# ruuda/robigo-luculenta

Hardware: AMD Instinct MI355X
Metric: Mrays/sec on built-in scene at 1920x1080 (higher is better)
Workload: dtype f32

## Files before the change

### robigo_luculenta_amd/csrc/rl_core.h

```cpp
#pragma once
#include "rl_math.h"
#include "rl_rng.h"
#include "rl_scene.h"

#if defined(__HIP_DEVICE_COMPILE__) && !defined(__gfx950__)
#error "rl_core.h's device fast paths (64-bit ballots, two scratch slots per lane, ds_bpermute batches) are written for wave64 gfx950"
#endif

struct RlF3 {
    float x, y, z;
};
RL_HD RlF3 rl_f3(float x, float y, float z) {
    RlF3 r;
    r.x = x;
    r.y = y;
    r.z = z;
    return r;
}
RL_HD RlF3 rl_add(RlF3 a, RlF3 b) { return rl_f3(a.x + b.x, a.y + b.y, a.z + b.z); }
RL_HD RlF3 rl_sub(RlF3 a, RlF3 b) { return rl_f3(a.x - b.x, a.y - b.y, a.z - b.z); }
RL_HD RlF3 rl_neg(RlF3 a) { return rl_f3(-a.x, -a.y, -a.z); }
RL_HD RlF3 rl_mul(RlF3 a, float f) { return rl_f3(a.x * f, a.y * f, a.z * f); }
RL_HD float rl_dot(RlF3 a, RlF3 b) { return a.x * b.x + a.y * b.y + a.z * b.z; }
RL_HD RlF3 rl_cross(RlF3 a, RlF3 b) {
// ... 61 lines not shown
RL_HD RlF3 rl_xyz(RlF4 v) { return rl_f3(v.x, v.y, v.z); }

struct RlQuat {
    float x, y, z, w;
};
RL_HD RlQuat rl_qmul(RlQuat a, RlQuat b) {
    RlQuat r;
    r.x = a.w * b.x + a.x * b.w + a.y * b.z - a.z * b.y;
    r.y = a.w * b.y - a.x * b.z + a.y * b.w + a.z * b.x;
    r.z = a.w * b.z + a.x * b.y - a.y * b.x + a.z * b.w;
    r.w = a.w * b.w - a.x * b.x - a.y * b.y - a.z * b.z;
    return r;
}
RL_HD RlF3 rl_qrotate(RlF3 v, RlQuat q) {
    RlQuat p;
    p.x = v.x; p.y = v.y; p.z = v.z; p.w = 0.0f;
    RlQuat c;
    c.x = -q.x; c.y = -q.y; c.z = -q.z; c.w = q.w;
    const RlQuat r = rl_qmul(rl_qmul(q, p), c);
    return rl_f3(r.x, r.y, r.z);
}


struct RlPath {
    RlF3 origin, direction;
    float wavelength;
    float intensity;
    float continue_chance;
    float sx, sy;
    float ior;
    uint32_t bounce;
};

enum { RL_HIT_NONE = 0xffffffffu };

struct RlHit {
    float t;
    uint32_t obj;
    uint32_t sub;
};

RL_HD float rl_sf10_ior(float wavelength) {
    const double w2 = (double)(wavelength * wavelength * 1.0e-6f);
#if defined(__HIP_DEVICE_COMPILE__)
    {
        const double t1 = w2 - 0.0131887070, t2 = w2 - 0.0623068142, t3 = w2 - 155.23629000;
        const double t23 = t2 * t3, t13 = t1 * t3, t12 = t1 * t2;
        const double num = __builtin_fma(1.737596950 * w2, t23, __builtin_fma(0.313747346 * w2, t13, (1.898781010 * w2) * t12));
        const double den = t1 * t23;
        double y = __builtin_amdgcn_rcp(den);
        y = __builtin_fma(y, __builtin_fma(-den, y, 1.0), y);
        y = __builtin_fma(y, __builtin_fma(-den, y, 1.0), y);
        const double sum = 1.0 + num * y;
        double r = __builtin_amdgcn_rsq(sum);
        r = __builtin_fma(0.5 * r, __builtin_fma(-(sum * r), r, 1.0), r);
        r = __builtin_fma(0.5 * r, __builtin_fma(-(sum * r), r, 1.0), r);
        const double n = sum * r;
        const float lo = (float)(n * (1.0 - 9.094947017729282e-13)), hi = (float)(n * (1.0 + 9.094947017729282e-13));
        if (RL_LIKELY(__builtin_amdgcn_ballot_w64(!(lo == hi)) == 0)) return lo;
    }
#endif
    return (float)sqrt(1.0 + 1.737596950 * w2 / (w2 - 0.0131887070) + 0.313747346 * w2 / (w2 - 0.0623068142) +
                       1.898781010 * w2 / (w2 - 155.23629000));
}


RL_HD void rl_begin_path(const RlSceneView& sv, float aspect_ratio, uint64_t seed, uint32_t stream, uint64_t path,
                         RlPath* p) {
    const RlRngBlock b0 = rl_rng_block(seed, stream, path, 0);
    const float wavelength = rl_get_wavelength(b0.w[0]);
    const float x = rl_get_bi_unit(b0.w[1]);
    const float y = rl_get_bi_unit(b0.w[2]) / aspect_ratio;
    const float t = rl_get_unit(b0.w[3]);

    const float* crec = (const float*)sv.camera_rec;
    RlCameraDesc cd;
    cd.phi0 = crec[0]; cd.phi1 = crec[1]; cd.alpha0 = crec[2]; cd.alpha1 = crec[3]; cd.dist0 = crec[4]; cd.dist1 = crec[5];
    cd.fov_over_pi = crec[6]; cd.focal_factor = crec[7]; cd.depth_of_field = crec[8]; cd.chromatic_abberation = crec[9];
    const float screen_distance = crec[10];
    const float phi = RL_PI_F * (cd.phi0 + cd.phi1 * t);
    const float alpha = RL_PI_F * (cd.alpha0 + cd.alpha1 * t);
    const float distance = cd.dist0 + cd.dist1 * t;
    float sin_a, cos_a, sin_p, cos_p;
    rl_sincosf(alpha, &sin_a, &cos_a);
    rl_sincosf(phi, &sin_p, &cos_p);
    const RlF3 position = rl_f3(cos_a * sin_p * distance, cos_a * cos_p * distance, sin_a * distance);
    float s1, c1, s2, c2;
    rl_sincosf((phi + RL_PI_F) * 0.5f, &s1, &c1);
    rl_sincosf((-alpha) * 0.5f, &s2, &c2);
    RlQuat q1, q2;
    q1.x = s1 * 0.0f; q1.y = s1 * 0.0f; q1.z = s1 * -1.0f; q1.w = c1;
    q2.x = s2 * 1.0f; q2.y = s2 * 0.0f; q2.z = s2 * 0.0f;  q2.w = c2;
    const RlQuat orientation = rl_qmul(q1, q2);
    const float focal_distance = distance * cd.focal_factor;

    const RlRngBlock b1 = rl_rng_block(seed, stream, path, 1);
    const float dof_angle = rl_get_longitude(b1.w[0]);
    const float dof_radius = rl_get_unit(b1.w[1]) / cd.depth_of_field;
    const float d = rl_div200f(wavelength - 580.0f);
    const float zoom = 1.0f + d * cd.chromatic_abberation;

    const float xs = x * zoom;
    const float ys = y * zoom;
    const RlF3 direction = rl_normalise(rl_f3(xs, screen_distance, -ys));
    const RlF3 focus_point = rl_mul(direction, focal_distance / direction.y);
    float sin_d, cos_d;
    rl_sincosf(dof_angle, &sin_d, &cos_d);
    const RlF3 lens_point = rl_f3(cos_d * dof_radius, 0.0f, sin_d * dof_radius);

    p->origin = rl_add(position, rl_qrotate(lens_point, orientation));
    p->direction = rl_normalise(rl_qrotate(rl_sub(focus_point, lens_point), orientation));
    p->wavelength = wavelength;
    p->intensity = 1.0f;
    p->continue_chance = 1.0f;
    p->sx = x;
    p->sy = y;
    p->ior = rl_sf10_ior(wavelength);
    p->bounce = 0;
}


template <bool AXIS_Z = false>
RL_HD float rl_plane_t(RlF3 n, RlF3 off, RlF3 o, RlF3 dir, float* dn_out) {
    const RlF3 lo = rl_sub(o, off);
    const float dn = AXIS_Z ? n.z * dir.z : rl_dot(n, dir);
    *dn_out = dn;
    const float t = -(AXIS_Z ? n.z * lo.z : rl_dot(n, lo)) / dn;
    return (dn != 0.0f && t > 0.0f) ? t : -1.0f;
}
template <bool AXIS_Z = false>
RL_HD bool rl_plane_hit(RlF3 n, RlF3 off, RlF3 o, RlF3 dir, float* t_out) {
    const RlF3 lo = rl_sub(o, off);
    const float dn = AXIS_Z ? n.z * dir.z : rl_dot(n, dir);
    const float t = -(AXIS_Z ? n.z * lo.z : rl_dot(n, lo)) / dn;
    *t_out = t;
    return (dn != 0.0f) & (t > 0.0f);
}
RL_HD bool rl_inside(RlF3 n, RlF3 off, RlF3 p) { return rl_dot(rl_sub(p, off), n) < 0.0f; }

RL_HD float rl_paraboloid_roots(float a, float b, float c) {
    if (a == 0.0f) {
        const float t1 = -c / b;
        if (t1 < 0.0f) return -1.0f;
        return t1;
    }
    const float disc = b * b - 4.0f * a * c;
    if (disc < 0.0f) return -1.0f;
    const float sq = sqrtf(disc);
    const float p = 0.5f * (-b + sq) / a;
    const float q = 0.5f * (-b - sq) / a;
    if (p > 0.0f && (p < q || q < 0.0f)) return p;
    if (q > 0.0f) return q;
    return -1.0f;
}
template <bool AXIS_Z = false>
RL_HD float rl_paraboloid_t(RlF3 offset, RlF3 normal, RlF3 focal_point, RlF3 o, RlF3 dir, bool* hit_out = nullptr) {
    const RlF3 origin = rl_sub(o, offset);
    const RlF3 focal_offset = rl_sub(origin, focal_point);
    const float n_dot_d = AXIS_Z ? normal.z * dir.z : rl_dot(normal, dir);
    const float n_dot_o = AXIS_Z ? normal.z * origin.z : rl_dot(normal, origin);
    const float d_dot_f = rl_dot(dir, focal_offset);
    const float a = n_dot_d * n_dot_d - 1.0f;
    const float b = 2.0f * n_dot_d * n_dot_o - 2.0f * d_dot_f;
    const float c = n_dot_o * n_dot_o - rl_dot(focal_offset, focal_offset);
#if defined(__HIP_DEVICE_COMPILE__)
    const float disc = b * b - 4.0f * a * c;
    const float sq = rl_sqrtf(disc, true);
    const float np = -b + sq, nq = -b - sq;
    const float pick = np < 0.0f ? np : nq;
    float largest;
    asm("v_max_f32 %0, |%1|, %2" : "=v"(largest) : "v"(b), "v"(sq));
    const bool plain = (a < 0.0f) & ((disc < 0.0f) | (largest >= 8.0779356694631609e-28f));
    if (RL_LIKELY(__builtin_amdgcn_ballot_w64(!plain) == 0)) {
        const float t = 0.5f * pick / a;
        if (hit_out) {
            *hit_out = !(disc < 0.0f) & (pick < 0.0f);
            return t;
        }
        return ((disc < 0.0f) | !(pick < 0.0f)) ? -1.0f : t;
    }
#endif
    const float t_literal = rl_paraboloid_roots(a, b, c);
    if (hit_out) *hit_out = !(t_literal < 0.0f);
    return t_literal;
}

struct RlCand {
    float t;
    uint32_t k;
};
// ... 629 lines not shown
```

### robigo_luculenta_amd/csrc/rl_kernels.hip.h

```cpp
#pragma once
#include <hip/hip_runtime.h>

#include <cstddef>
#include <type_traits>

#include "rl_cie1931.h"
#include "rl_core.h"

#define RL_BLOCK 256
#ifndef RL_TRACE_BLOCK
#define RL_TRACE_BLOCK 1024
#endif
#ifndef RL_TRACE_WPS
#define RL_TRACE_WPS 4
#endif
#ifndef RL_TRACE_VGPRS
#define RL_TRACE_VGPRS (RL_TRACE_WPS == 4 ? 128 : 96)
#endif
#ifndef RL_TRACE_VGPRS_OPEN
#define RL_TRACE_VGPRS_OPEN (RL_TRACE_WPS == 4 ? 120 : 96)
#endif
#define RL_EMIT_MAX_AGE 8u
#define RL_CHUNK 256ull

// ... 1022 lines not shown
        if (pend_me) __hip_atomic_fetch_add(wg_fin + my_job, 1u, __ATOMIC_RELAXED, __HIP_MEMORY_SCOPE_WORKGROUP);
        if (lane < emit_pend)
            __hip_atomic_fetch_add(wg_fin + (((RlLdsU32*)ws->ring_b)[lane] >> 24), 1u, __ATOMIC_RELAXED,
                                   __HIP_MEMORY_SCOPE_WORKGROUP);
        pend_me = false;
        pend_any = false;
        emit_pend = 0;
    };
    auto flush = [&](uint32_t gap) {
        const uint32_t now = (uint32_t)wall_clock64();
        uint32_t mine = gap == 0u ? 1u : 0u;
        if (lane == 0 && gap != 0u) {
            uint32_t at = *wg_flushed_at;
            if (now - at >= gap)
                mine = __hip_atomic_compare_exchange_strong(wg_flushed_at, &at, now | 1u, __ATOMIC_RELAXED, __ATOMIC_RELAXED,
                                                            __HIP_MEMORY_SCOPE_WORKGROUP) ? 1u : 0u;
        }
        if (__builtin_amdgcn_readfirstlane(mine) == 0u) return;
        for (uint32_t base_job = 0; base_job < known_local; base_job += 64u) {
            const uint32_t jb = base_job + lane;
            uint32_t f = 0, sg = 0;
            if (jb < known_local) {
                f = __hip_atomic_exchange(wg_fin + jb, 0u, __ATOMIC_RELAXED, __HIP_MEMORY_SCOPE_WORKGROUP);
                sg = __hip_atomic_exchange(wg_seg + jb, 0u, __ATOMIC_RELAXED, __HIP_MEMORY_SCOPE_WORKGROUP);
            }
            if (__builtin_amdgcn_ballot_w64((f | sg) != 0u) == 0) continue;
            if (sg != 0) __hip_atomic_fetch_add(&od->seg[jb], sg, __ATOMIC_RELAXED, __HIP_MEMORY_SCOPE_AGENT);
            __builtin_amdgcn_fence(__ATOMIC_RELEASE, "workgroup");
            if (f != 0) {
                const uint32_t before = __hip_atomic_fetch_add(&od->fin[jb], f, __ATOMIC_RELAXED, __HIP_MEMORY_SCOPE_AGENT);
                if (before + f == (uint32_t)od->jobs[jb].end) {
                    __hip_atomic_fetch_add(&od->completed, 1u, __ATOMIC_RELAXED, __HIP_MEMORY_SCOPE_AGENT);
                    const uint32_t total = __hip_atomic_load(&od->seg[jb], __ATOMIC_RELAXED, __HIP_MEMORY_SCOPE_AGENT);
                    __hip_atomic_store(&ctl->segs[jb], total, __ATOMIC_RELAXED, __HIP_MEMORY_SCOPE_SYSTEM);
                    __hip_atomic_store(&ctl->done[jb], 1u, __ATOMIC_RELEASE, __HIP_MEMORY_SCOPE_SYSTEM);
                }
            }
        }
    };
    uint32_t e_head = 0, e_tail = 0;
    uint32_t emit_age = 0;
#ifdef RL_STATS
    unsigned long long st[RL_ST_COUNT];
    for (int k = 0; k < RL_ST_COUNT; ++k) st[k] = 0;
#endif
    RL_T0(t_total);

    auto process_emitted = [&](uint32_t count) {
        RL_STAT(RL_ST_EMIT_BATCHES, 1);
        RL_STAT(RL_ST_EMIT_LANES, count);
        if (OPEN && emit_pend != 0) settle();
        rl_wave_sync();
        if (!FUSED) {
            uint32_t idx = 0, tagged = 0;
            float value = 0.0f;
            RlMappedPhoton* dst_base = photons;
            if (lane < count) {
                const uint32_t slot = (e_head + lane) & 63u;
                idx = rl_f2u(emit_get(0, slot));
                tagged = rl_f2u(emit_get(4, slot));
                if (OPEN) ((RlLdsU32*)ws->ring_b)[lane] = tagged;
                uint64_t first = job.first_path;
                if (OPEN) {
                    const RlJobEntry e = jobs[tagged >> 24];
                    first = e.first_path, dst_base = (RlMappedPhoton*)e.target;
                }
                const RlRngBlock b0 = rl_rng_block(job.seed, job.stream, first + idx, 0);
                RlMappedPhoton ph;
                ph.wavelength = rl_get_wavelength(b0.w[0]);
                ph.x = rl_get_bi_unit(b0.w[1]);
                ph.y = rl_get_bi_unit(b0.w[2]) / job.aspect_ratio;
                value = rl_emission(sv, emit_get(3, slot), ph.wavelength, OPEN ? (tagged & 0xffffffu) : tagged);
                ph.probability = value;
                if (OPEN) {
                    uint32_t* dst = (uint32_t*)&dst_base[idx];
                    __hip_atomic_store(dst + 0, rl_f2u(ph.x), __ATOMIC_RELAXED, __HIP_MEMORY_SCOPE_AGENT);
                    __hip_atomic_store(dst + 1, rl_f2u(ph.y), __ATOMIC_RELAXED, __HIP_MEMORY_SCOPE_AGENT);
                    __hip_atomic_store(dst + 2, rl_f2u(ph.probability), __ATOMIC_RELAXED, __HIP_MEMORY_SCOPE_AGENT);
                    __hip_atomic_store(dst + 3, rl_f2u(ph.wavelength), __ATOMIC_RELAXED, __HIP_MEMORY_SCOPE_AGENT);
                } else {
                    dst_base[idx] = ph;
                }
            }
        } else if (lane < count) {
            const uint32_t slot = (e_head + lane) & 63u;
            const float sx = emit_get(0, slot), sy = emit_get(1, slot), wavelength = emit_get(2, slot);
            const uint32_t tagged = rl_f2u(emit_get(4, slot));
            if (OPEN) ((RlLdsU32*)ws->ring_b)[lane] = tagged;
            float* target = plot;
            if (OPEN) target = (float*)jobs[tagged >> 24].target;
            const float value = rl_emission(sv, emit_get(3, slot), wavelength, OPEN ? (tagged & 0xffffffu) : tagged);
            if (value != 0.0f) {
                const RlF3 cie = rl_mul(rl_tristimulus(sv.cie, wavelength), value);
                uint32_t width = job.width, height = job.height;
                asm volatile("" : "+s"(width), "+s"(height));
                const RlSplat sp = rl_splat_weights(width, height, job.wm1, job.hm1, job.aspect_ratio, sx, sy);
#pragma unroll
                for (int k = 0; k < 4; ++k) {
                    float* px = target + 3ull * sp.idx[k];
                    unsafeAtomicAdd(px + 0, cie.x * sp.w[k]);
                    unsafeAtomicAdd(px + 1, cie.y * sp.w[k]);
                    unsafeAtomicAdd(px + 2, cie.z * sp.w[k]);
                }
            }
        }
        if (OPEN) emit_pend = count;
        rl_wave_sync();
    };

    for (;;) {
        if (OPEN) {
            settle();
            flush(3000u);
        }
        RL_T0(t_refill);
        auto refill = [&]() -> bool {
            if (drained) return false;
                uint32_t open_n = 0;
                if (OPEN) {
                    bool got = false;
                    for (;;) {
                        if (chunk_next < chunk_end) {
                            open_n = (uint32_t)jobs[stash_job].end;
                            got = true;
                            break;
                        }
                        if (stash_job < known_local) {
                            open_n = (uint32_t)jobs[stash_job].end;
                            const uint32_t take = known_local - stash_job >= 2u ? 256u : 64u;
                            uint32_t b = 0;
                            if (lane == 0) b = __hip_atomic_fetch_add(&od->next[stash_job], take, __ATOMIC_RELAXED, __HIP_MEMORY_SCOPE_AGENT);
                            b = __builtin_amdgcn_readfirstlane(b);
                            if (b < open_n) {
                                chunk_end = b + take < open_n ? b + take : ((open_n + 63u) & ~63u);
                                chunk_next = b;
                                got = true;
                                break;
                            }
                            stash_job += 1u;
                            continue;
                        }
                        const uint32_t now = (uint32_t)wall_clock64();
                        const uint32_t seen = __builtin_amdgcn_readfirstlane(wg_poll[0]), seen_at = __builtin_amdgcn_readfirstlane(wg_poll[1]);
                        if (seen > known_local) {
                            __builtin_amdgcn_fence(__ATOMIC_ACQUIRE, "agent");
                            known_local = seen;
                            continue;
                        }
                        if (now - seen_at < 1000u) break;
                        if (lane == 0) wg_poll[1] = now;
                        uint32_t v = 0;
                        if (lane == 0) v = __hip_atomic_load(&od->known, __ATOMIC_RELAXED, __HIP_MEMORY_SCOPE_AGENT);
                        v = __builtin_amdgcn_readfirstlane(v);
                        if (v > known_local) {
                            if (lane == 0) wg_poll[0] = v;
                            __builtin_amdgcn_fence(__ATOMIC_ACQUIRE, "agent");
                            known_local = v;
                            continue;
                        }
                        if (lane == 0) v = __hip_atomic_load(&od->closed, __ATOMIC_RELAXED, __HIP_MEMORY_SCOPE_AGENT);
                        if (__builtin_amdgcn_readfirstlane(v) != 0u) {
                            drained = true;
                            break;
                        }
                        if (lane == 0) {
                            uint32_t expected = 0;
                            v = __hip_atomic_compare_exchange_strong(&od->closing, &expected, 1u, __ATOMIC_ACQUIRE, __ATOMIC_RELAXED,
                                                                     __HIP_MEMORY_SCOPE_AGENT) ? 1u : 0u;
                        }
                        if (__builtin_amdgcn_readfirstlane(v) == 0u) break;
                        uint32_t pub = 0;
                        if (lane == 0) pub = __hip_atomic_load(&ctl->published, __ATOMIC_ACQUIRE, __HIP_MEMORY_SCOPE_SYSTEM);
                        pub = __builtin_amdgcn_readfirstlane(pub);
                        if (pub > RL_OPEN_CAP) pub = RL_OPEN_CAP;
                        if (pub > known_local) {
                            for (uint32_t k = known_local + lane; k < pub; k += 64u) {
                                unsigned long long* dst = (unsigned long long*)&od->jobs[k];
                                const unsigned long long* src = (const unsigned long long*)&ctl->jobs[k];
                                for (int w = 0; w < 4; ++w)
                                    __hip_atomic_store(dst + w, __hip_atomic_load(src + w, __ATOMIC_RELAXED, __HIP_MEMORY_SCOPE_SYSTEM),
                                                       __ATOMIC_RELAXED, __HIP_MEMORY_SCOPE_AGENT);
                            }
                            __builtin_amdgcn_fence(__ATOMIC_RELEASE, "agent");
                            if (lane == 0) {
                                od->idle_since = 0;
                                od->stuck_since = 0;
                                wg_poll[0] = pub;
                                __hip_atomic_store(&od->known, pub, __ATOMIC_RELEASE, __HIP_MEMORY_SCOPE_AGENT);
                                __hip_atomic_store(&od->closing, 0u, __ATOMIC_RELEASE, __HIP_MEMORY_SCOPE_AGENT);
                            }
                            known_local = pub;
                            continue;
                        }
                        uint32_t stay = 0;
                        if (lane == 0 && known_local < RL_OPEN_CAP) {
                            const bool finishing = __hip_atomic_load(&od->completed, __ATOMIC_RELAXED, __HIP_MEMORY_SCOPE_AGENT) < known_local;
                            const unsigned long long now = wall_clock64(), since = finishing ? od->stuck_since : od->idle_since;
                            uint32_t grace = job.grace_ticks;
                            asm volatile("" : "+s"(grace));
                            const unsigned long long limit = finishing ? 500000000ull : (unsigned long long)grace;
                            if (since == 0) (finishing ? od->stuck_since : od->idle_since) = now, stay = 1;
                            else if (now - since < limit) stay = 1;
                            if (!finishing) od->stuck_since = 0;
                            if (stay) __hip_atomic_store(&od->closing, 0u, __ATOMIC_RELEASE, __HIP_MEMORY_SCOPE_AGENT);
                        }
                        if (__builtin_amdgcn_readfirstlane(stay) != 0u) break;
                        uint32_t again = 0;
                        if (lane == 0) {
                            __hip_atomic_store(&ctl->closed_at, known_local, __ATOMIC_SEQ_CST, __HIP_MEMORY_SCOPE_SYSTEM);
                            __builtin_amdgcn_fence(__ATOMIC_SEQ_CST, "");
                            again = __hip_atomic_load(&ctl->published, __ATOMIC_SEQ_CST, __HIP_MEMORY_SCOPE_SYSTEM);
                        }
                        again = __builtin_amdgcn_readfirstlane(again);
                        if (again == known_local || known_local >= RL_OPEN_CAP) {
                            if (lane == 0) {
                                __hip_atomic_store(&ctl->final_at, known_local, __ATOMIC_SEQ_CST, __HIP_MEMORY_SCOPE_SYSTEM);
                                __hip_atomic_store(&od->closed, 1u, __ATOMIC_RELEASE, __HIP_MEMORY_SCOPE_AGENT);
                            }
                            drained = true;
                            break;
                        }
                        if (lane == 0) {
                            __hip_atomic_store(&ctl->closed_at, RL_OPEN_NONE, __ATOMIC_SEQ_CST, __HIP_MEMORY_SCOPE_SYSTEM);
                            __hip_atomic_store(&od->closing, 0u, __ATOMIC_RELEASE, __HIP_MEMORY_SCOPE_AGENT);
                        }
                    }
                    if (!got) return false;
                }
                if (!OPEN && chunk_next == chunk_end) {
                    const unsigned long long chunk =
                        job.n_paths >= (unsigned long long)gridDim.x * (RL_TRACE_BLOCK * 16ull) ? RL_CHUNK : 64ull;
                    unsigned long long b = 0;
                    if (lane == 0) b = atomicAdd(&queue[0], chunk);
                    const uint32_t lo = __builtin_amdgcn_readfirstlane((uint32_t)b);
                    const uint32_t hi = __builtin_amdgcn_readfirstlane((uint32_t)(b >> 32));
                    chunk_next = ((uint64_t)hi << 32) | lo;
                    chunk_end = chunk_next + chunk;
                }
                RL_STAT(RL_ST_REFILLS, 1);
                if (OPEN) stash_first = jobs[stash_job].first_path;
                const uint64_t limit = OPEN ? (uint64_t)open_n : job.n_paths;
                stash_path0 = stash_first + chunk_next;
                stash_valid = chunk_next >= limit ? 0u : (limit - chunk_next >= 64ull ? 64u : (uint32_t)(limit - chunk_next));
                chunk_next += 64;
                const bool valid = lane < stash_valid;
                const uint64_t path_index = stash_path0 + lane;
                RlPath fresh = p;
                RL_T0(t_cam);
                if (valid) rl_begin_path(sv, job.aspect_ratio, job.seed, job.stream, path_index, &fresh);
                RL_T1(RL_ST_T_CAMERA, t_cam);
                rl_wave_sync();
                stash[0 * 64 + lane] = fresh.origin.x;
                stash[1 * 64 + lane] = fresh.origin.y;
                stash[2 * 64 + lane] = fresh.origin.z;
                stash[3 * 64 + lane] = fresh.direction.x;
                stash[4 * 64 + lane] = fresh.direction.y;
                stash[5 * 64 + lane] = fresh.direction.z;
                stash[6 * 64 + lane] = fresh.wavelength;
                stash[7 * 64 + lane] = fresh.sx;
                stash[8 * 64 + lane] = fresh.sy;
                stash[9 * 64 + lane] = fresh.ior;
                rl_wave_sync();
                stash_head = 0;
                stash_count = 64;
                if (!OPEN && chunk_next >= job.n_paths) drained = true;
            return true;
        };
        auto hand_out = [&](const uint64_t need) -> bool {
            const uint32_t avail = stash_count - stash_head;
            const uint32_t rank = rl_mbcnt(need);
            const uint32_t slot = stash_head + rank;
            const bool take = !active & (rank < avail) & (slot < stash_valid);
            {
                const uint32_t sl = slot & 63u;
                const float s0 = stash[0 * 64 + sl], s1 = stash[1 * 64 + sl], s2 = stash[2 * 64 + sl], s3 = stash[3 * 64 + sl], s4 = stash[4 * 64 + sl];
                const float s5 = stash[5 * 64 + sl], s6 = stash[6 * 64 + sl], s7 = stash[7 * 64 + sl], s8 = stash[8 * 64 + sl], s9 = stash[9 * 64 + sl];
                my_path = take ? stash_path0 + slot : my_path;
                if (OPEN) my_job = take ? stash_job : my_job;
                p.origin = rl_f3(take ? s0 : p.origin.x, take ? s1 : p.origin.y, take ? s2 : p.origin.z);
                p.direction = rl_f3(take ? s3 : p.direction.x, take ? s4 : p.direction.y, take ? s5 : p.direction.z);
                p.wavelength = take ? s6 : p.wavelength;
                p.sx = take ? s7 : p.sx;
                p.sy = take ? s8 : p.sy;
                p.ior = take ? s9 : p.ior;
                p.intensity = take ? 1.0f : p.intensity;
                p.continue_chance = take ? 1.0f : p.continue_chance;
                p.bounce = take ? 0u : p.bounce;
                active = active | take;
            }
            const uint32_t wanted = (uint32_t)__popcll(need);
            stash_head += wanted < avail ? wanted : avail;
            return wanted <= avail;
        };
        {
            const uint64_t need = __builtin_amdgcn_ballot_w64(!active);
            if (need != 0) {
                bool served = false;
                if (RL_LIKELY(stash_count != stash_head)) served = hand_out(need);
                if (RL_UNLIKELY(!served)) {
                    if (refill()) hand_out(__builtin_amdgcn_ballot_w64(!active));
                }
            }
        }
        RL_T1(RL_ST_T_REFILL, t_refill);
        if (__builtin_amdgcn_ballot_w64(active) == 0) {
            if (!OPEN || drained) break;
            settle();
            if (e_tail != e_head) {
                process_emitted(e_tail - e_head);
                e_head = e_tail;
                settle();
            }
            flush(500u);
            for (int k = 0; k < 4; ++k) __builtin_amdgcn_s_sleep(127);
            continue;
        }
        constexpr bool FULL = !OPEN || (STAGE == RL_STAGE_ALL && (FUSED || !CYL));
        const RlHit hit = rl_scan_wave<CYL, FULL, STAGE != RL_STAGE_NONE && (!(FUSED && OPEN) || FULL), STAGE != RL_STAGE_NONE && (!(OPEN && (FUSED || STAGE == RL_STAGE_TABLES)) || FULL), STAGE == RL_STAGE_ALL, STAGE != RL_STAGE_NONE, STAGE != RL_STAGE_ALL>(sv, base + (lay.off_cull - tab0), CYL ? base + (lay.off_prism_cyl - tab0) : nullptr, lay.group_gc, lay.small_ordered, lay.cull_cmax2, lay.n_cluster_groups, lay.n_prism_groups,
                                       lay.n_cluster_supers, lay.super_g, ring_t, p.origin, p.direction, active ? 0u : 0x80000000u, ws, lane RL_TACC_ARG);
#ifdef RL_STATS
        {
            const uint32_t mk = (active && hit.obj != RL_HIT_NONE) ? rl_object_material(rl_f2u(sv.objects[hit.obj].w)) : 99u;
            const uint64_t m_act = __builtin_amdgcn_ballot_w64(active);
            const uint64_t m_void = __builtin_amdgcn_ballot_w64(active && hit.obj == RL_HIT_NONE);
            const uint64_t m_emit = __builtin_amdgcn_ballot_w64(mk == RL_MATERIAL_BLACK_BODY);
            const uint64_t m_grey = __builtin_amdgcn_ballot_w64(mk == RL_MATERIAL_DIFFUSE_GREY);
            const uint64_t m_col = __builtin_amdgcn_ballot_w64(mk == RL_MATERIAL_DIFFUSE_COLOURED);
            const uint64_t m_gls = __builtin_amdgcn_ballot_w64(mk == RL_MATERIAL_GLOSSY_MIRROR);
            const uint64_t m_glass = __builtin_amdgcn_ballot_w64(mk == RL_MATERIAL_SF10_GLASS);
            const uint64_t m_soap = __builtin_amdgcn_ballot_w64(mk == RL_MATERIAL_SOAP_BUBBLE);
            RL_STAT(RL_ST_ITER, 1);
            RL_STAT(RL_ST_SCAN_LANES, __popcll(m_act));
            RL_STAT(RL_ST_END_VOID, __popcll(m_void));
            RL_STAT(RL_ST_END_EMITTER, __popcll(m_emit));
            RL_STAT(RL_ST_SHADE_DIFFUSE, __popcll(m_grey | m_col | m_gls));
            RL_STAT(RL_ST_SHADE_GLASS, __popcll(m_glass));
            RL_STAT(RL_ST_SHADE_SOAP, __popcll(m_soap));
            RL_STAT(RL_ST_ANY_DIFFUSE, (m_grey | m_col | m_gls) != 0);
            RL_STAT(RL_ST_ANY_GLASS, m_glass != 0);
            RL_STAT(RL_ST_ANY_SOAP, m_soap != 0);
            RL_STAT(RL_ST_ANY_COLOURED, m_col != 0);
            RL_STAT(RL_ST_ANY_GLOSSY, m_gls != 0);
        }
#endif
        RL_T0(t_shade);
        bool ended_on_emitter = false, ended_now = false;
        uint32_t emit_obj = 0, emit_idx = 0;
        if (active) {
            segments += 1;
            float value;
            uint32_t emitter = 0;
            const int status = rl_bounce(sv, job.seed, job.stream, my_path, &p, hit, &value, &emitter);
            if (status != RL_PATH_CONTINUES) {
                active = false;
                p.direction = rl_f3(0.0f, 0.0f, 0.0f);
                paths_done += 1;
                ended_on_emitter = status == RL_PATH_ENDED_ON_EMITTER;
                emit_obj = OPEN ? (emitter | (my_job << 24)) : emitter;
                if (!FUSED && !ended_on_emitter) {
                    RlMappedPhoton ph;
                    ph.x = p.sx;
                    ph.y = p.sy;
                    ph.probability = value;
                    ph.wavelength = p.wavelength;
                    if (OPEN) {
                        const RlJobEntry e = jobs[my_job];
                        uint32_t* dst = (uint32_t*)&((RlMappedPhoton*)e.target)[my_path - e.first_path];
                        __hip_atomic_store(dst + 0, rl_f2u(ph.x), __ATOMIC_RELAXED, __HIP_MEMORY_SCOPE_AGENT);
                        __hip_atomic_store(dst + 1, rl_f2u(ph.y), __ATOMIC_RELAXED, __HIP_MEMORY_SCOPE_AGENT);
                        __hip_atomic_store(dst + 2, rl_f2u(ph.probability), __ATOMIC_RELAXED, __HIP_MEMORY_SCOPE_AGENT);
                        __hip_atomic_store(dst + 3, rl_f2u(ph.wavelength), __ATOMIC_RELAXED, __HIP_MEMORY_SCOPE_AGENT);
                    } else {
                        photons[my_path - job.first_path] = ph;
                    }
                }
                if (!FUSED && ended_on_emitter) emit_idx = (uint32_t)(my_path - (OPEN ? jobs[my_job].first_path : job.first_path));
                if (OPEN) {
                    ended_now = true;
                    __hip_atomic_fetch_add(wg_seg + my_job, p.bounce + ((hit.obj == RL_HIT_NONE || status == RL_PATH_ENDED_ON_EMITTER) ? 1u : 0u),
                                           __ATOMIC_RELAXED, __HIP_MEMORY_SCOPE_WORKGROUP);
                }
            }
        }
        if (OPEN) {
            pend_me = ended_now && !ended_on_emitter;
            pend_any = __builtin_amdgcn_ballot_w64(pend_me) != 0;
            ended_now = false;
        }
        RL_T1(RL_ST_T_SHADE, t_shade);
        RL_T0(t_emit);
        {
            const uint64_t m = __builtin_amdgcn_ballot_w64(ended_on_emitter);
            if (m != 0) {
                const uint32_t n_new = (uint32_t)__popcll(m);
                if (RL_UNLIKELY(e_tail - e_head + n_new > 64u)) {
                    process_emitted(e_tail - e_head);
                    e_head = e_tail;
                }
                if (ended_on_emitter) {
                    const uint32_t slot = rl_mbcnt_from(m, e_tail) & 63u;
                    if (FUSED) {
                        emit_put(0, slot, p.sx);
                        emit_put(1, slot, p.sy);
                        emit_put(2, slot, p.wavelength);
                    } else {
                        emit_put(0, slot, rl_u2f(emit_idx));
                    }
                    emit_put(3, slot, p.intensity);
                    emit_put(4, slot, rl_u2f(emit_obj));
                    ended_on_emitter = false;
                }
                e_tail += n_new;
                if (RL_UNLIKELY(e_tail - e_head == 64u)) {
                    process_emitted(64u);
                    e_head += 64u;
                }
            }
            if (OPEN && !FUSED) {
                emit_age = e_tail != e_head ? emit_age + 1u : 0u;
                if (RL_UNLIKELY(emit_age >= RL_EMIT_MAX_AGE)) {
                    process_emitted(e_tail - e_head);
                    e_head = e_tail;
                    emit_age = 0;
                }
            }
        }
        RL_T1(RL_ST_T_EMIT, t_emit);
    }
    if (e_tail != e_head) process_emitted(e_tail - e_head);
    if (OPEN) {
        settle();
        flush(0u);
    }
    RL_T1(RL_ST_T_TOTAL, t_total);
#ifdef RL_STATS
    if (lane == 0)
        for (int k = 0; k < RL_ST_COUNT; ++k) atomicAdd(&rl_stat_counters[k], st[k]);
#endif
    uint32_t s = segments, d = paths_done;
#pragma unroll
    for (int off = 32; off > 0; off >>= 1) {
        s += __shfl_down(s, off);
        d += __shfl_down(d, off);
    }
    if (lane == 0) {
        atomicAdd(&queue[1], (unsigned long long)s);
        atomicAdd(&queue[2], (unsigned long long)d);
    }
}

template <int STAGE, bool FUSED, bool CYL>
__global__ __launch_bounds__(RL_TRACE_BLOCK, RL_TRACE_WPS) __attribute__((amdgpu_num_vgpr(RL_TRACE_VGPRS / 2))) void rl_trace_kernel(const RlF4* __restrict__ scene, RlSceneLayout lay, RlTraceJob job,
                                                                                                       RlMappedPhoton* __restrict__ photons, float* __restrict__ plot,
                                                                                                       unsigned long long* __restrict__ queue, const RlJobEntry* jobs,
                                                                                                       RlOpenDev* od, RlOpenCtl* ctl) {
    rl_trace_body<STAGE, FUSED, false, CYL>(scene, lay, job, photons, plot, queue, jobs, od, ctl);
}
template <int STAGE, bool FUSED, bool CYL>
__global__ __launch_bounds__(RL_TRACE_BLOCK, RL_TRACE_WPS) __attribute__((amdgpu_num_vgpr(RL_TRACE_VGPRS_OPEN / 2))) void rl_trace_kernel_open(const RlF4* __restrict__ scene, RlSceneLayout lay, RlTraceJob job,
                                                                                                            RlMappedPhoton* __restrict__ photons, float* __restrict__ plot,
                                                                                                            unsigned long long* __restrict__ queue, const RlJobEntry* jobs,
                                                                                                            RlOpenDev* od, RlOpenCtl* ctl) {
    rl_trace_body<STAGE, FUSED, true, CYL>(scene, lay, job, photons, plot, queue, jobs, od, ctl);
}

__global__ __launch_bounds__(RL_BLOCK) void rl_plot_kernel(const RlMappedPhoton* __restrict__ photons, uint32_t n,
                                                           const RlF4* __restrict__ cie, uint32_t width, uint32_t height,
                                                           float aspect_ratio, float* __restrict__ plot) {
    __shared__ RlF4 s_cie[RL_CIE_SAMPLES];
    for (uint32_t i = threadIdx.x; i < RL_CIE_SAMPLES; i += RL_BLOCK) s_cie[i] = cie[i];
    __syncthreads();
    for (uint32_t i = blockIdx.x * RL_BLOCK + threadIdx.x; i < n; i += gridDim.x * RL_BLOCK) {
        const RlMappedPhoton ph = photons[i];
        if (ph.probability == 0.0f) continue;
        const RlF3 c = rl_mul(rl_tristimulus(s_cie, ph.wavelength), ph.probability);
        const RlSplat s = rl_splat_weights(width, height, aspect_ratio, ph.x, ph.y);
#pragma unroll
        for (int k = 0; k < 4; ++k) {
            float* px = plot + 3ull * s.idx[k];
            unsafeAtomicAdd(px + 0, c.x * s.w[k]);
            unsafeAtomicAdd(px + 1, c.y * s.w[k]);
            unsafeAtomicAdd(px + 2, c.z * s.w[k]);
        }
    }
}

__global__ __launch_bounds__(RL_BLOCK) void rl_gather_kernel(float* __restrict__ acc, float* __restrict__ comp,
// ... 223 lines not shown
```

### robigo_luculenta_amd/csrc/rl_math.h

```cpp
#pragma once
#define RL_LIKELY(X) __builtin_expect(!!(X), 1)
#define RL_UNLIKELY(X) __builtin_expect(!!(X), 0)
#include <stdint.h>
#include <math.h>

#if defined(__HIPCC__)
#include <hip/hip_runtime.h>
#define RL_HD __host__ __device__ __forceinline__
#else
#define RL_HD inline
#endif

#define RL_PI_F 3.14159274101257324f

RL_HD uint64_t rl_bits_d(double x) { return __builtin_bit_cast(uint64_t, x); }
RL_HD double rl_from_bits_d(uint64_t b) { return __builtin_bit_cast(double, b); }
RL_HD uint32_t rl_bits_f(float x) { return __builtin_bit_cast(uint32_t, x); }
RL_HD float rl_from_bits_f(uint32_t b) { return __builtin_bit_cast(float, b); }
RL_HD double rl_horner_d(double p, double x, double c) {
#if defined(__HIP_DEVICE_COMPILE__)
    if (!__builtin_constant_p(c)) return __builtin_fma(p, x, c);
    double r;
    asm("v_fma_f64 %0, %1, %2, %3" : "=v"(r) : "v"(p), "v"(x), "s"(c));
    return r;
#else
    return __builtin_fma(p, x, c);
#endif
}

RL_HD float rl_fmaf(float a, float b, float c) { return __builtin_fmaf(a, b, c); }

RL_HD float rl_sqrtf(float x, bool magnitude_only = false) {
#if defined(__HIP_DEVICE_COMPILE__)
    const float a = magnitude_only ? fabsf(x) : x;
    const bool in_range = rl_bits_f(a) - 0x0f800000u < 0x7f800000u - 0x0f800000u;
    if (RL_LIKELY(__builtin_amdgcn_ballot_w64(!in_range) == 0)) {
        const float y = __builtin_amdgcn_rsqf(a);
        const float s = a * y, h = 0.5f * y;
        return __builtin_fmaf(__builtin_fmaf(-s, s, a), h, s);
    }
#endif
    return sqrtf(magnitude_only ? fabsf(x) : x);
}

RL_HD void rl_sincos_core_d(double x, double* sr_out, double* cr_out, int* k_out) {
    const double TWO_OVER_PI = 0.6366197723675814;
    const double PIO2_1 = 1.5707963267341256;
    const double PIO2_1T = 6.077100506506192e-11;
    const double kd = floor(x * TWO_OVER_PI + 0.5);
    const double r = (x - kd * PIO2_1) - kd * PIO2_1T;
    *k_out = (int)kd;
    const double z = r * r;
    double ps = 2.8114572543455206e-15;
    ps = rl_horner_d(ps, z, -7.647163731819816e-13);
    ps = rl_horner_d(ps, z, 1.6059043836821613e-10);
    ps = rl_horner_d(ps, z, -2.505210838544172e-08);
    ps = rl_horner_d(ps, z, 2.7557319223985893e-06);
    ps = rl_horner_d(ps, z, -0.0001984126984126984);
    ps = rl_horner_d(ps, z, 0.008333333333333333);
    ps = rl_horner_d(ps, z, -0.16666666666666666);
    *sr_out = r + r * (z * ps);
    double pc = -1.5619206968586225e-16;
    pc = rl_horner_d(pc, z, 4.779477332387385e-14);
    pc = rl_horner_d(pc, z, -1.1470745597729725e-11);
    pc = rl_horner_d(pc, z, 2.08767569878681e-09);
    pc = rl_horner_d(pc, z, -2.755731922398589e-07);
    pc = rl_horner_d(pc, z, 2.48015873015873e-05);
    pc = rl_horner_d(pc, z, -0.001388888888888889);
    pc = rl_horner_d(pc, z, 0.041666666666666664);
    pc = rl_horner_d(pc, z, -0.5);
    *cr_out = 1.0 + z * pc;
}
RL_HD void rl_sincos_d(double x, double* s_out, double* c_out) {
    double sr, cr;
    int k;
    rl_sincos_core_d(x, &sr, &cr, &k);
    const int q = k & 3;
    const double s = (q & 1) ? cr : sr;
    const double c = (q & 1) ? sr : cr;
    *s_out = (q & 2) ? -s : s;
    *c_out = ((q + 1) & 2) ? -c : c;
}

RL_HD void rl_sincosf_d(float x, float* s_out, float* c_out) {
    double sr, cr;
    int k;
    rl_sincos_core_d((double)x, &sr, &cr, &k);
    const float sf = (float)sr, cf = (float)cr;
    const int q = k & 3;
    const float s = (q & 1) ? cf : sf;
    const float c = (q & 1) ? sf : cf;
    *s_out = (q & 2) ? -s : s;
    *c_out = ((q + 1) & 2) ? -c : c;
}
RL_HD void rl_sincosf(float x, float* s_out, float* c_out) {
    if (!(fabsf(x) <= 32.0f)) {
        rl_sincosf_d(x, s_out, c_out);
        return;
    }
    const float TWO_OVER_PI = 0.636619746685028076171875f;
    const float P1 = 1.5703125f;
    const float P2 = 4.83751296997070312e-04f;
    const float P3 = 7.54979012640433211e-08f;
    const float P4 = -1.71512449944288301e-15f;
    const float kf = floorf(x * TWO_OVER_PI + 0.5f);
    const float r0 = rl_fmaf(-kf, P1, x);
    const float r1 = rl_fmaf(-kf, P2, r0);
    const float ph = kf * P3;
    const float pl = rl_fmaf(kf, P3, -ph);
    const float r = r1 - ph;
    const float er = (r1 - r) - ph;
    const float rl = rl_fmaf(-kf, P4, er - pl);
    const int k = (int)kf;
    const float z = r * r;
    const float rz = r * z;
    float ps = 2.7248365768173244e-06f;
    ps = rl_fmaf(ps, z, -0.00019840073946397752f);
    ps = rl_fmaf(ps, z, 0.008333331905305386f);
    ps = rl_fmaf(ps, z, -0.1666666716337204f);
    float pc = 2.454665445839055e-05f;
    pc = rl_fmaf(pc, z, -0.001388829667121172f);
    pc = rl_fmaf(pc, z, 0.0416666641831398f);
    const float hz = 0.5f * z;
    const float w = 1.0f - hz;
    const float sa = rl_fmaf(rz, -0.16666667163372039795f, r);
    const float cf = w + (((1.0f - w) - hz) + rl_fmaf(z * z, pc, -(sa * rl)));
    const float sf = r + rl_fmaf(rz, ps, rl * w);
    const int q = k & 3;
    const float s = (q & 1) ? cf : sf;
    const float c = (q & 1) ? sf : cf;
    *s_out = (q & 2) ? -s : s;
    *c_out = ((q + 1) & 2) ? -c : c;
}
RL_HD float rl_sinf(float x) {
    float s, c;
    rl_sincosf(x, &s, &c);
    return s;
}
RL_HD float rl_cosf(float x) {
    float s, c;
    rl_sincosf(x, &s, &c);
    return c;
}
RL_HD float rl_sinf_d(float x) {
    float s, c;
    rl_sincosf_d(x, &s, &c);
    return s;
}
RL_HD float rl_cosf_d(float x) {
    float s, c;
    rl_sincosf_d(x, &s, &c);
    return c;
}
RL_HD float rl_tanf(float x) {
    double s, c;
    rl_sincos_d((double)x, &s, &c);
    return (float)(s / c);
}

RL_HD double rl_exp_core_d(double x, int* k_out) {
    const double LOG2E = 1.4426950408889634;
    const double LN2_HI = 0.6931471803691238;
    const double LN2_LO = 1.9082149292705877e-10;
    const double kd = floor(x * LOG2E + 0.5);
    const double r = (x - kd * LN2_HI) - kd * LN2_LO;
    double p = 1.1470745597729725e-11;
    p = rl_horner_d(p, r, 1.6059043836821613e-10);
    p = rl_horner_d(p, r, 2.08767569878681e-09);
    p = rl_horner_d(p, r, 2.505210838544172e-08);
    p = rl_horner_d(p, r, 2.755731922398589e-07);
    p = rl_horner_d(p, r, 2.7557319223985893e-06);
    p = rl_horner_d(p, r, 2.48015873015873e-05);
    p = rl_horner_d(p, r, 0.0001984126984126984);
    p = rl_horner_d(p, r, 0.001388888888888889);
    p = rl_horner_d(p, r, 0.008333333333333333);
    p = rl_horner_d(p, r, 0.041666666666666664);
    p = rl_horner_d(p, r, 0.16666666666666666);
    p = rl_horner_d(p, r, 0.5);
    *k_out = (int)kd;
    return 1.0 + (r + (r * r) * p);
}
RL_HD double rl_exp_d(double x) {
    if (x < -745.0) return 0.0;
    if (x > 709.0) return rl_from_bits_d(0x7ff0000000000000ull);
    int k;
    const double e = rl_exp_core_d(x, &k);
    const int k1 = k / 2;
    const int k2 = k - k1;
    const double s1 = rl_from_bits_d((uint64_t)(k1 + 1023) << 52);
    const double s2 = rl_from_bits_d((uint64_t)(k2 + 1023) << 52);
    return (e * s1) * s2;
}
RL_HD float rl_expf_d(float x) {
    if (!(x >= -86.0f && x <= 88.0f)) return (float)rl_exp_d((double)x);
    int k;
    const float e = (float)rl_exp_core_d((double)x, &k);
    return ldexpf(e, k);
}
RL_HD float rl_expf(float x) {
    if (!(x >= -86.0f && x <= 88.0f)) return (float)rl_exp_d((double)x);
    const float LOG2E = 1.44269502162933349609375f;
    const float LN2_HI = 0.693145751953125f;
    const float LN2_LO = 1.42860676533018704e-06f;
    const float kf = floorf(x * LOG2E + 0.5f);
    const float rh = rl_fmaf(-kf, LN2_HI, x);
    const float r = rl_fmaf(-kf, LN2_LO, rh);
    float p = 0.00019891103147529066f;
    p = rl_fmaf(p, r, 0.0013933751033619046f);
    p = rl_fmaf(p, r, 0.00833331048488617f);
    p = rl_fmaf(p, r, 0.041666463017463684f);
    p = rl_fmaf(p, r, 0.1666666716337204f);
    p = rl_fmaf(p, r, 0.5f);
    const float e = 1.0f + rl_fmaf(r * r, p, r);
    return ldexpf(e, (int)kf);
}

RL_HD double rl_log_d(double x) {
    const double LN2_HI = 0.6931471803691238;
    const double LN2_LO = 1.9082149292705877e-10;
    const uint64_t b = rl_bits_d(x);
    int e = (int)(b >> 52) - 1023;
    double m = rl_from_bits_d((b & 0x000fffffffffffffull) | 0x3ff0000000000000ull);
    if (m > 1.4142135623730951) {
        m = m * 0.5;
        e = e + 1;
    }
    const double s = (m - 1.0) / (m + 1.0);
    const double z = s * s;
    double p = 0.047619047619047616;
    p = rl_horner_d(p, z, 0.05263157894736842);
    p = rl_horner_d(p, z, 0.058823529411764705);
    p = rl_horner_d(p, z, 0.06666666666666667);
    p = rl_horner_d(p, z, 0.07692307692307693);
    p = rl_horner_d(p, z, 0.09090909090909091);
    p = rl_horner_d(p, z, 0.1111111111111111);
    p = rl_horner_d(p, z, 0.14285714285714285);
    p = rl_horner_d(p, z, 0.2);
    p = rl_horner_d(p, z, 0.3333333333333333);
    const double lm = 2.0 * s + 2.0 * s * (z * p);
    const double ed = (double)e;
    return ed * LN2_HI + (lm + ed * LN2_LO);
}
RL_HD float rl_logf(float x) { return (float)rl_log_d((double)x); }

RL_HD float rl_powf(float x, float y) { return (float)rl_exp_d((double)y * rl_log_d((double)x)); }

RL_HD float rl_logf_full(float x) {
    if (x != x) return x;
    if (x < 0.0f) return rl_from_bits_f(0x7fc00000u);
    if (x == 0.0f) return rl_from_bits_f(0xff800000u);
    if (x == rl_from_bits_f(0x7f800000u)) return x;
    return (float)rl_log_d((double)x);
}
RL_HD float rl_powf_full(float x, float y) {
    if (x != x) return x;
    if (x == 0.0f) return 0.0f;
    if (x == rl_from_bits_f(0x7f800000u)) return x;
    return rl_powf(x, y);
}
RL_HD uint8_t rl_to_u8(float x) { return (x != x) ? (uint8_t)0 : (uint8_t)x; }

RL_HD double rl_asin_core_d(double y) {
    const double z = y * y;
    double p = 0.027921912047656466;
    p = rl_horner_d(p, z, -0.0029555479088451027);
    p = rl_horner_d(p, z, 0.015682585691969324);
    p = rl_horner_d(p, z, 0.013186282871554133);
    p = rl_horner_d(p, z, 0.017441719105456513);
    p = rl_horner_d(p, z, 0.022366048091739782);
    p = rl_horner_d(p, z, 0.030382183571536783);
    p = rl_horner_d(p, z, 0.044642852420329455);
    p = rl_horner_d(p, z, 0.07500000003599422);
    p = rl_horner_d(p, z, 0.1666666666666216);
    return y + y * (z * p);
}
RL_HD double rl_acos_d(double x) {
    const double PI = 3.141592653589793;
    const double PIO2 = 1.5707963267948966;
    const double ax = x < 0.0 ? -x : x;
    const bool big = ax > 0.5;
    double y = x;
    if (big) y = sqrt((1.0 - ax) * 0.5);
    const double a = rl_asin_core_d(y);
    if (!big) return PIO2 - a;
    return x < 0.0 ? PI - 2.0 * a : 2.0 * a;
}
RL_HD float rl_acosf_d(float x) { return (float)rl_acos_d((double)x); }
RL_HD float rl_acosf(float x) {
    const float PIO2_HI = 1.57079625129699707031f;
    const float PIO2_LO = 7.54978995489188194e-08f;
    const float ax = fabsf(x);
    const bool big = ax > 0.5f;
    const float zb = (1.0f - ax) * 0.5f;
    const float z = big ? zb : x * x;
    const float y = big ? rl_sqrtf(zb) : x;
    float p = 0.03370072692632675f;
    p = rl_fmaf(p, z, 0.017143717035651207f);
// ... 11 lines not shown
```

### robigo_luculenta_amd/csrc/rl_rng.h

```cpp
#pragma once
#include "rl_math.h"

struct RlRngBlock {
    uint32_t w[4];
};

RL_HD uint32_t rl_mulhi32(uint32_t a, uint32_t b) { return (uint32_t)(((uint64_t)a * (uint64_t)b) >> 32); }

#define RL_PHILOX_ROUNDS 7
template <int ROUNDS, bool UNIFORM_KEY = false>
RL_HD RlRngBlock rl_philox4x32(uint32_t c0, uint32_t c1, uint32_t c2, uint32_t c3, uint32_t k0, uint32_t k1) {
    const uint32_t M0 = 0xD2511F53u, M1 = 0xCD9E8D57u, W0 = 0x9E3779B9u, W1 = 0xBB67AE85u;
#if defined(__HIP_DEVICE_COMPILE__)
    if (UNIFORM_KEY) asm volatile("" : "+s"(k0), "+s"(k1));
#endif
#if defined(__HIPCC__)
#pragma unroll
#endif
    for (int round = 0; round < ROUNDS; ++round) {
#if defined(__HIP_DEVICE_COMPILE__)
        unsigned long long p0, p1, carry;
        asm("v_mad_u64_u32 %0, %1, %2, %3, 0" : "=v"(p0), "=s"(carry) : "v"(c0), "s"(M0));
        asm("v_mad_u64_u32 %0, %1, %2, %3, 0" : "=v"(p1), "=s"(carry) : "v"(c2), "s"(M1));
        const uint32_t hi0 = (uint32_t)(p0 >> 32), lo0 = (uint32_t)p0;
        const uint32_t hi1 = (uint32_t)(p1 >> 32), lo1 = (uint32_t)p1;
#else
        const uint32_t hi0 = rl_mulhi32(M0, c0), lo0 = M0 * c0;
        const uint32_t hi1 = rl_mulhi32(M1, c2), lo1 = M1 * c2;
#endif
        const uint32_t n0 = hi1 ^ c1 ^ k0;
        const uint32_t n2 = hi0 ^ c3 ^ k1;
        c0 = n0;
        c1 = lo1;
        c2 = n2;
        c3 = lo0;
        k0 += W0;
        k1 += W1;
    }
    RlRngBlock r;
    r.w[0] = c0;
    r.w[1] = c1;
    r.w[2] = c2;
    r.w[3] = c3;
    return r;
}

RL_HD RlRngBlock rl_philox4x32_10(uint32_t c0, uint32_t c1, uint32_t c2, uint32_t c3, uint32_t k0, uint32_t k1) {
    return rl_philox4x32<10>(c0, c1, c2, c3, k0, k1);
}

RL_HD RlRngBlock rl_rng_block(uint64_t seed, uint32_t stream, uint64_t path, uint32_t block) {
    return rl_philox4x32<RL_PHILOX_ROUNDS, true>((uint32_t)path, (uint32_t)(path >> 32), block, stream, (uint32_t)seed,
                                           (uint32_t)(seed >> 32));
}

RL_HD float rl_halfopen01(uint32_t u) { return (float)(u >> 8) * 5.9604644775390625e-8f; }
RL_HD float rl_closed01(uint32_t u) { return rl_halfopen01(u) * (16777216.0f / 16777215.0f); }

RL_HD float rl_get_unit(uint32_t u) { return rl_closed01(u); }
RL_HD float rl_get_bi_unit(uint32_t u) { return rl_closed01(u) * 2.0f - 1.0f; }
RL_HD float rl_get_longitude(uint32_t u) { return rl_halfopen01(u) * RL_PI_F * 2.0f; }
RL_HD float rl_get_wavelength(uint32_t u) { return rl_closed01(u) * 400.0f + 380.0f; }
```

Measured before the change: 22360.

## Recompute splat coords from path RNG, wave-uniform sincos/exp fallbacks, bitop3 philox

Stops carrying sx/sy/wavelength through the stash and the emit ring in the fused path. It stores the 64-bit path id instead and regenerates these values from the Philox block when splatting. Sincos and exp now take the short polynomial path unconditionally and run the double-precision fallback only when a wave ballot finds an out-of-range lane, which removes per-lane divergent branches. Philox XOR chains use a 3-input bitop3. Together these reduce LDS traffic and live registers, at the cost of extra Philox rounds per emitted photon and recomputation done by all lanes.

Result: no change. 22570 (median of 6 runs) (+0.9%).

```diff
diff --git a/robigo_luculenta_amd/csrc/rl_core.h b/robigo_luculenta_amd/csrc/rl_core.h
--- a/robigo_luculenta_amd/csrc/rl_core.h
+++ b/robigo_luculenta_amd/csrc/rl_core.h
@@ -167,12 +167,34 @@
     const float alpha = RL_PI_F * (cd.alpha0 + cd.alpha1 * t);
     const float distance = cd.dist0 + cd.dist1 * t;
     float sin_a, cos_a, sin_p, cos_p;
+    float s1, c1, s2, c2;
+    const float half_phi = (phi + RL_PI_F) * 0.5f, half_alpha = (-alpha) * 0.5f;
+#if defined(__HIP_DEVICE_COMPILE__)
+    rl_sincosf_short(alpha, &sin_a, &cos_a);
+    rl_sincosf_short(phi, &sin_p, &cos_p);
+    rl_sincosf_short(half_phi, &s1, &c1);
+    rl_sincosf_short(half_alpha, &s2, &c2);
+    if (RL_UNLIKELY(__builtin_amdgcn_ballot_w64(rl_sincosf_far(alpha) | rl_sincosf_far(phi)) != 0)) {
+#pragma nounroll
+        for (int i = 0; i < 4; ++i) {
+            const float a = i == 0 ? alpha : (i == 1 ? phi : (i == 2 ? half_phi : half_alpha));
+            if (rl_sincosf_far(a)) {
+                float s, c;
+                rl_sincosf_d(a, &s, &c);
+                sin_a = i == 0 ? s : sin_a, cos_a = i == 0 ? c : cos_a;
+                sin_p = i == 1 ? s : sin_p, cos_p = i == 1 ? c : cos_p;
+                s1 = i == 2 ? s : s1, c1 = i == 2 ? c : c1;
+                s2 = i == 3 ? s : s2, c2 = i == 3 ? c : c2;
+            }
+        }
+    }
+#else
     rl_sincosf(alpha, &sin_a, &cos_a);
     rl_sincosf(phi, &sin_p, &cos_p);
+    rl_sincosf(half_phi, &s1, &c1);
+    rl_sincosf(half_alpha, &s2, &c2);
+#endif
     const RlF3 position = rl_f3(cos_a * sin_p * distance, cos_a * cos_p * distance, sin_a * distance);
-    float s1, c1, s2, c2;
-    rl_sincosf((phi + RL_PI_F) * 0.5f, &s1, &c1);
-    rl_sincosf((-alpha) * 0.5f, &s2, &c2);
     RlQuat q1, q2;
     q1.x = s1 * 0.0f; q1.y = s1 * 0.0f; q1.z = s1 * -1.0f; q1.w = c1;
     q2.x = s2 * 1.0f; q2.y = s2 * 0.0f; q2.z = s2 * 0.0f;  q2.w = c2;
@@ -190,7 +212,11 @@
     const RlF3 direction = rl_normalise(rl_f3(xs, screen_distance, -ys));
     const RlF3 focus_point = rl_mul(direction, focal_distance / direction.y);
     float sin_d, cos_d;
+#if defined(__HIP_DEVICE_COMPILE__)
+    rl_sincosf_short(dof_angle, &sin_d, &cos_d);
+#else
     rl_sincosf(dof_angle, &sin_d, &cos_d);
+#endif
     const RlF3 lens_point = rl_f3(cos_d * dof_radius, 0.0f, sin_d * dof_radius);
 
     p->origin = rl_add(position, rl_qrotate(lens_point, orientation));
diff --git a/robigo_luculenta_amd/csrc/rl_kernels.hip.h b/robigo_luculenta_amd/csrc/rl_kernels.hip.h
--- a/robigo_luculenta_amd/csrc/rl_kernels.hip.h
+++ b/robigo_luculenta_amd/csrc/rl_kernels.hip.h
@@ -1128,25 +1128,30 @@
                     dst_base[idx] = ph;
                 }
             }
-        } else if (lane < count) {
+        } else {
             const uint32_t slot = (e_head + lane) & 63u;
-            const float sx = emit_get(0, slot), sy = emit_get(1, slot), wavelength = emit_get(2, slot);
-            const uint32_t tagged = rl_f2u(emit_get(4, slot));
-            if (OPEN) ((RlLdsU32*)ws->ring_b)[lane] = tagged;
-            float* target = plot;
-            if (OPEN) target = (float*)jobs[tagged >> 24].target;
-            const float value = rl_emission(sv, emit_get(3, slot), wavelength, OPEN ? (tagged & 0xffffffu) : tagged);
-            if (value != 0.0f) {
-                const RlF3 cie = rl_mul(rl_tristimulus(sv.cie, wavelength), value);
-                uint32_t width = job.width, height = job.height;
-                asm volatile("" : "+s"(width), "+s"(height));
-                const RlSplat sp = rl_splat_weights(width, height, job.wm1, job.hm1, job.aspect_ratio, sx, sy);
+            const uint64_t path = ((uint64_t)rl_f2u(emit_get(1, slot)) << 32) | rl_f2u(emit_get(0, slot));
+            const RlRngBlock b0 = rl_rng_block_rare(job.seed, job.stream, path, 0);
+            if (lane < count) {
+                const float wavelength = rl_get_wavelength(b0.w[0]);
+                const float sx = rl_get_bi_unit(b0.w[1]), sy = rl_get_bi_unit(b0.w[2]) / job.aspect_ratio;
+                const uint32_t tagged = rl_f2u(emit_get(4, slot));
+                if (OPEN) ((RlLdsU32*)ws->ring_b)[lane] = tagged;
+                float* target = plot;
+                if (OPEN) target = (float*)jobs[tagged >> 24].target;
+                const float value = rl_emission(sv, emit_get(3, slot), wavelength, OPEN ? (tagged & 0xffffffu) : tagged);
+                if (value != 0.0f) {
+                    const RlF3 cie = rl_mul(rl_tristimulus(sv.cie, wavelength), value);
+                    uint32_t width = job.width, height = job.height;
+                    asm volatile("" : "+s"(width), "+s"(height));
+                    const RlSplat sp = rl_splat_weights(width, height, job.wm1, job.hm1, job.aspect_ratio, sx, sy);
 #pragma unroll
-                for (int k = 0; k < 4; ++k) {
-                    float* px = target + 3ull * sp.idx[k];
-                    unsafeAtomicAdd(px + 0, cie.x * sp.w[k]);
-                    unsafeAtomicAdd(px + 1, cie.y * sp.w[k]);
-                    unsafeAtomicAdd(px + 2, cie.z * sp.w[k]);
+                    for (int k = 0; k < 4; ++k) {
+                        float* px = target + 3ull * sp.idx[k];
+                        unsafeAtomicAdd(px + 0, cie.x * sp.w[k]);
+                        unsafeAtomicAdd(px + 1, cie.y * sp.w[k]);
+                        unsafeAtomicAdd(px + 2, cie.z * sp.w[k]);
+                    }
                 }
             }
         }
@@ -1303,9 +1308,13 @@
                 stash[4 * 64 + lane] = fresh.direction.y;
                 stash[5 * 64 + lane] = fresh.direction.z;
                 stash[6 * 64 + lane] = fresh.wavelength;
-                stash[7 * 64 + lane] = fresh.sx;
-                stash[8 * 64 + lane] = fresh.sy;
-                stash[9 * 64 + lane] = fresh.ior;
+                if (FUSED) {
+                    stash[7 * 64 + lane] = fresh.ior;
+                } else {
+                    stash[7 * 64 + lane] = fresh.sx;
+                    stash[8 * 64 + lane] = fresh.sy;
+                    stash[9 * 64 + lane] = fresh.ior;
+                }
                 rl_wave_sync();
                 stash_head = 0;
                 stash_count = 64;
@@ -1320,14 +1329,17 @@
             {
                 const uint32_t sl = slot & 63u;
                 const float s0 = stash[0 * 64 + sl], s1 = stash[1 * 64 + sl], s2 = stash[2 * 64 + sl], s3 = stash[3 * 64 + sl], s4 = stash[4 * 64 + sl];
-                const float s5 = stash[5 * 64 + sl], s6 = stash[6 * 64 + sl], s7 = stash[7 * 64 + sl], s8 = stash[8 * 64 + sl], s9 = stash[9 * 64 + sl];
+                const float s5 = stash[5 * 64 + sl], s6 = stash[6 * 64 + sl], s7 = stash[7 * 64 + sl];
+                const float s8 = FUSED ? 0.0f : stash[8 * 64 + sl], s9 = FUSED ? s7 : stash[9 * 64 + sl];
                 my_path = take ? stash_path0 + slot : my_path;
                 if (OPEN) my_job = take ? stash_job : my_job;
                 p.origin = rl_f3(take ? s0 : p.origin.x, take ? s1 : p.origin.y, take ? s2 : p.origin.z);
                 p.direction = rl_f3(take ? s3 : p.direction.x, take ? s4 : p.direction.y, take ? s5 : p.direction.z);
                 p.wavelength = take ? s6 : p.wavelength;
-                p.sx = take ? s7 : p.sx;
-                p.sy = take ? s8 : p.sy;
+                if (!FUSED) {
+                    p.sx = take ? s7 : p.sx;
+                    p.sy = take ? s8 : p.sy;
+                }
                 p.ior = take ? s9 : p.ior;
                 p.intensity = take ? 1.0f : p.intensity;
                 p.continue_chance = take ? 1.0f : p.continue_chance;
@@ -1446,9 +1458,8 @@
                 if (ended_on_emitter) {
                     const uint32_t slot = rl_mbcnt_from(m, e_tail) & 63u;
                     if (FUSED) {
-                        emit_put(0, slot, p.sx);
-                        emit_put(1, slot, p.sy);
-                        emit_put(2, slot, p.wavelength);
+                        emit_put(0, slot, rl_u2f((uint32_t)my_path));
+                        emit_put(1, slot, rl_u2f((uint32_t)(my_path >> 32)));
                     } else {
                         emit_put(0, slot, rl_u2f(emit_idx));
                     }
diff --git a/robigo_luculenta_amd/csrc/rl_math.h b/robigo_luculenta_amd/csrc/rl_math.h
--- a/robigo_luculenta_amd/csrc/rl_math.h
+++ b/robigo_luculenta_amd/csrc/rl_math.h
@@ -93,11 +93,8 @@
     *s_out = (q & 2) ? -s : s;
     *c_out = ((q + 1) & 2) ? -c : c;
 }
-RL_HD void rl_sincosf(float x, float* s_out, float* c_out) {
-    if (!(fabsf(x) <= 32.0f)) {
-        rl_sincosf_d(x, s_out, c_out);
-        return;
-    }
+RL_HD bool rl_sincosf_far(float x) { return !(fabsf(x) <= 32.0f); }
+RL_HD void rl_sincosf_short(float x, float* s_out, float* c_out) {
     const float TWO_OVER_PI = 0.636619746685028076171875f;
     const float P1 = 1.5703125f;
     const float P2 = 4.83751296997070312e-04f;
@@ -132,6 +129,21 @@
     *s_out = (q & 2) ? -s : s;
     *c_out = ((q + 1) & 2) ? -c : c;
 }
+RL_HD void rl_sincosf(float x, float* s_out, float* c_out) {
+#if defined(__HIP_DEVICE_COMPILE__)
+    rl_sincosf_short(x, s_out, c_out);
+    const bool far = rl_sincosf_far(x);
+    if (RL_UNLIKELY(__builtin_amdgcn_ballot_w64(far) != 0)) {
+        if (far) rl_sincosf_d(x, s_out, c_out);
+    }
+#else
+    if (rl_sincosf_far(x)) {
+        rl_sincosf_d(x, s_out, c_out);
+        return;
+    }
+    rl_sincosf_short(x, s_out, c_out);
+#endif
+}
 RL_HD float rl_sinf(float x) {
     float s, c;
     rl_sincosf(x, &s, &c);
@@ -197,8 +209,8 @@
     const float e = (float)rl_exp_core_d((double)x, &k);
     return ldexpf(e, k);
 }
-RL_HD float rl_expf(float x) {
-    if (!(x >= -86.0f && x <= 88.0f)) return (float)rl_exp_d((double)x);
+RL_HD bool rl_expf_far(float x) { return !(x >= -86.0f && x <= 88.0f); }
+RL_HD float rl_expf_short(float x) {
     const float LOG2E = 1.44269502162933349609375f;
     const float LN2_HI = 0.693145751953125f;
     const float LN2_LO = 1.42860676533018704e-06f;
@@ -213,6 +225,19 @@
     p = rl_fmaf(p, r, 0.5f);
     const float e = 1.0f + rl_fmaf(r * r, p, r);
     return ldexpf(e, (int)kf);
+}
+RL_HD float rl_expf(float x) {
+#if defined(__HIP_DEVICE_COMPILE__)
+    float e = rl_expf_short(x);
+    const bool far = rl_expf_far(x);
+    if (RL_UNLIKELY(__builtin_amdgcn_ballot_w64(far) != 0)) {
+        if (far) e = (float)rl_exp_d((double)x);
+    }
+    return e;
+#else
+    if (rl_expf_far(x)) return (float)rl_exp_d((double)x);
+    return rl_expf_short(x);
+#endif
 }
 
 RL_HD double rl_log_d(double x) {
diff --git a/robigo_luculenta_amd/csrc/rl_rng.h b/robigo_luculenta_amd/csrc/rl_rng.h
--- a/robigo_luculenta_amd/csrc/rl_rng.h
+++ b/robigo_luculenta_amd/csrc/rl_rng.h
@@ -8,11 +8,12 @@
 RL_HD uint32_t rl_mulhi32(uint32_t a, uint32_t b) { return (uint32_t)(((uint64_t)a * (uint64_t)b) >> 32); }
 
 #define RL_PHILOX_ROUNDS 7
-template <int ROUNDS, bool UNIFORM_KEY = false>
+template <int ROUNDS, bool UNIFORM_KEY = false, bool VECTOR_KEY = false>
 RL_HD RlRngBlock rl_philox4x32(uint32_t c0, uint32_t c1, uint32_t c2, uint32_t c3, uint32_t k0, uint32_t k1) {
     const uint32_t M0 = 0xD2511F53u, M1 = 0xCD9E8D57u, W0 = 0x9E3779B9u, W1 = 0xBB67AE85u;
 #if defined(__HIP_DEVICE_COMPILE__)
     if (UNIFORM_KEY) asm volatile("" : "+s"(k0), "+s"(k1));
+    if (VECTOR_KEY) asm volatile("" : "+v"(k0), "+v"(k1));
 #endif
 #if defined(__HIPCC__)
 #pragma unroll
@@ -28,8 +29,13 @@
         const uint32_t hi0 = rl_mulhi32(M0, c0), lo0 = M0 * c0;
         const uint32_t hi1 = rl_mulhi32(M1, c2), lo1 = M1 * c2;
 #endif
+#if defined(__HIP_DEVICE_COMPILE__)
+        const uint32_t n0 = __builtin_amdgcn_bitop3_b32(hi1, c1, k0, 0x96);
+        const uint32_t n2 = round == 0 ? hi0 ^ (c3 ^ k1) : __builtin_amdgcn_bitop3_b32(hi0, c3, k1, 0x96);
+#else
         const uint32_t n0 = hi1 ^ c1 ^ k0;
         const uint32_t n2 = hi0 ^ c3 ^ k1;
+#endif
         c0 = n0;
         c1 = lo1;
         c2 = n2;
@@ -54,6 +60,11 @@
                                            (uint32_t)(seed >> 32));
 }
 
+RL_HD RlRngBlock rl_rng_block_rare(uint64_t seed, uint32_t stream, uint64_t path, uint32_t block) {
+    return rl_philox4x32<RL_PHILOX_ROUNDS, false, true>((uint32_t)path, (uint32_t)(path >> 32), block, stream, (uint32_t)seed,
+                                                  (uint32_t)(seed >> 32));
+}
+
 RL_HD float rl_halfopen01(uint32_t u) { return (float)(u >> 8) * 5.9604644775390625e-8f; }
 RL_HD float rl_closed01(uint32_t u) { return rl_halfopen01(u) * (16777216.0f / 16777215.0f); }
 
```
